# stdio2016/pfann

Measured on AMD Instinct MI355X. Metric: query segments/sec, 10 s @ SNR 0 queries vs 1M-segment db (exact flat IP top-100 + sequence match), higher is better.
Workload: dtype f32

## Files before the change

### pfann_amd/csrc/search_f16.hip

```cpp
#include "search_common.h"
#include <stdlib.h>

namespace pfann {

typedef _Float16 f16x8 __attribute__((ext_vector_type(8)));

__global__ void rows_to_half_kernel(const float *__restrict__ x, int64_t n, int d, _Float16 *__restrict__ xh,
                                    float *norm_max) {
    const int lane = threadIdx.x & 63;
    const int64_t row = (int64_t)blockIdx.x * (blockDim.x >> 6) + (threadIdx.x >> 6);
    if (row >= n) return;
    float ss = 0.f;
    for (int e = lane; e < d; e += 64) {
        const float v = x[row * d + e];
        xh[row * d + e] = (_Float16)v;
        ss = fmaf(v, v, ss);
    }
    ss = wave_sum(ss);
    if (lane == 0) atomicMax(reinterpret_cast<unsigned *>(norm_max), __float_as_uint(sqrtf(ss)));
}

int launch_rows_to_half(const float *x, int64_t n, int d, void *xh, float *norm_max_dev, hipStream_t s) {
    if (n <= 0) return 0;
    PF_LAUNCH(rows_to_half_kernel, dim3((unsigned)cdiv(n, 4)), dim3(256), 0, s, x, n, d,
// ... 46 lines not shown
    for (int i = tid; i < QT * BM; i += 256) {
        const int64_t m = (int64_t)mt0 * BM + i;
        thr_s[i] = dense ? 0.f : (m < p.nq ? -p.thr[m] : -INFINITY);
    }
    const char *qb = reinterpret_cast<const char *>(p.q), *dbb = reinterpret_cast<const char *>(p.db);
    const int64_t mq0 = (int64_t)mt0 * BM;
    const __amdgpu_buffer_rsrc_t srd_q = make_srd(qb + mq0 * row_bytes, (unsigned long long)(p.nq - mq0) * row_bytes);
    __amdgpu_buffer_rsrc_t srd_db[BR];
    unsigned doff[BR];
#pragma unroll
    for (int j = 0; j < BR; ++j) {
        const int64_t nj = n0 + 32 * j;
        const int64_t left = p.nrows - nj;
        srd_db[j] = make_srd(dbb + (nj < p.nrows ? nj : 0) * p.row_stride * row_bytes,
                             left > 0 ? (unsigned long long)((left - 1) * p.row_stride + 1) * row_bytes : 0ull);
        doff[j] = nj + rowq < p.nrows ? (unsigned)((unsigned long long)rowq * p.row_stride * row_bytes) : BUF_OOB;
    }
    f32x4 ra[AR], rb[BR];
    const int q_rows_left = (int)((p.nq - mq0) < (int64_t)QT * BM ? (p.nq - mq0) : (int64_t)QT * BM);
    const unsigned tile_bytes = (unsigned)BM * row_bytes;
    unsigned aoff[AR];
#pragma unroll
    for (int i = 0; i < AR; ++i) aoff[i] = (unsigned)(rowq + 32 * i) * row_bytes;
    unsigned lkb = (unsigned)col4 * 16u;
    int lrow = rowq;
    unsigned lbase = 0;
    auto load_tile = [&]() {
        const bool kok = lkb < row_bytes;
#pragma unroll
        for (int i = 0; i < AR; ++i)
            ra[i] = buf_load4(srd_q, (kok && lrow + 32 * i < q_rows_left) ? lbase + aoff[i] + lkb : BUF_OOB);
#pragma unroll
        for (int j = 0; j < BR; ++j) rb[j] = buf_load4(srd_db[j], (kok && doff[j] != BUF_OOB) ? doff[j] + lkb : BUF_OOB);
        lkb += 128u;
        const bool wrap = lkb >= row_bytes;
        lkb = wrap ? (unsigned)col4 * 16u : lkb;
        lrow += wrap ? BM : 0;
        lbase += wrap ? tile_bytes : 0u;
    };
    auto store_tile = [&](float *Ad, float *Bd) {
#pragma unroll
        for (int i = 0; i < AR; ++i)
            *reinterpret_cast<f32x4 *>(&Ad[(rowq + 32 * i) * LDK + col4 * 4]) = ra[i];
#pragma unroll
        for (int j = 0; j < BR; ++j)
            *reinterpret_cast<f32x4 *>(&Bd[(rowq + 32 * j) * LDK + col4 * 4]) = rb[j];
    };

    const int nk = (int)((row_bytes + 127u) / 128u);
    load_tile();
    store_tile(As, Bs);
    __syncthreads();
    const int l31 = lane & 31, lhalf = lane >> 5;
    int it = 0;
#pragma unroll 1
    for (int q = 0; q < n_q; ++q) {
        const int64_t m0 = mq0 + (int64_t)q * BM;
        const float *thr_c = thr_s + q * BM;
        f32x16 acc[TM][TN];
#pragma unroll
        for (int i = 0; i < TM; ++i)
#pragma unroll
            for (int g = 0; g < 4; ++g) {
                const f32x4 t4 = *reinterpret_cast<const f32x4 *>(thr_c + wm * WM + i * 32 + 8 * g + 4 * lhalf);
#pragma unroll
                for (int j = 0; j < TN; ++j)
#pragma unroll
                    for (int e = 0; e < 4; ++e) acc[i][j][4 * g + e] = t4[e];
            }
#pragma unroll 1
        for (int kt = 0; kt < nk; ++kt, ++it) {
            const float *Ac = As + (it & 1) * (BM * LDK), *Bc = Bs + (it & 1) * (BN * LDK);
            float *An = As + ((it + 1) & 1) * (BM * LDK), *Bn = Bs + ((it + 1) & 1) * (BN * LDK);
#pragma unroll
            for (int kk = 0; kk < 4; ++kk) {
                f16x8 a8[TM], b8[TN];
#pragma unroll
                for (int i = 0; i < TM; ++i)
                    a8[i] = __builtin_bit_cast(f16x8, *reinterpret_cast<const f32x4 *>(
                                                          &Ac[(wm * WM + i * 32 + l31) * LDK + kk * 8 + lhalf * 4]));
#pragma unroll
                for (int j = 0; j < TN; ++j)
                    b8[j] = __builtin_bit_cast(f16x8, *reinterpret_cast<const f32x4 *>(
                                                          &Bc[(wn * WN + j * 32 + l31) * LDK + kk * 8 + lhalf * 4]));
                if (kk == 0) {
                    load_tile();
                    __builtin_amdgcn_sched_barrier(0);
                }
                if (kk == 3) store_tile(An, Bn);
#pragma unroll
                for (int i = 0; i < TM; ++i)
#pragma unroll
                    for (int j = 0; j < TN; ++j)
                        acc[i][j] = __builtin_amdgcn_mfma_f32_32x32x16_f16(a8[i], b8[j], acc[i][j], 0, 0, 0);
            }
            __syncthreads();
        }
        if constexpr (EXCL) {
            if (excl_span_hit(p.excl_tile[m0 >> 7], n0 * p.row_stride, (n0 + BN - 1) * p.row_stride)) {
#pragma unroll
                for (int i = 0; i < TM; ++i)
#pragma unroll
                    for (int r = 0; r < 16; ++r) {
                        const int64_t m = m0 + wm * WM + i * 32 + (r & 3) + 8 * (r >> 2) + 4 * lhalf;
                        const uint2 ex = m < p.nq ? p.excl[m] : make_uint2(0u, 0u);
#pragma unroll
                        for (int j = 0; j < TN; ++j)
                            if (excl_hit(ex, (unsigned)((n0 + wn * WN + j * 32 + l31) * p.row_stride))) acc[i][j][r] = -INFINITY;
                    }
            }
        }
#pragma unroll
        for (int j = 0; j < TN; ++j) {
            const int64_t n = n0 + wn * WN + j * 32 + l31;
            const bool nok = n < p.nrows;
            const unsigned row = (unsigned)(n * p.row_stride);
#pragma unroll
            for (int i = 0; i < TM; ++i) {
                if (EXCL && dense) {
#pragma unroll
                    for (int r = 0; r < 16; ++r) {
                        const int64_t m = m0 + wm * WM + i * 32 + (r & 3) + 8 * (r >> 2) + 4 * lhalf;
                        if (nok && m < p.nq && acc[i][j][r] != -INFINITY)
                            p.keys[m * CAP + atomicAdd(&p.cnt[m], 1)] = pack_key(acc[i][j][r], row);
                    }
                } else if (dense) {
#pragma unroll
                    for (int r = 0; r < 16; ++r) {
                        const int64_t m = m0 + wm * WM + i * 32 + (r & 3) + 8 * (r >> 2) + 4 * lhalf;
                        if (nok && m < p.nq) p.keys[m * CAP + n] = pack_key(acc[i][j][r], row);
                    }
                } else {
                    float mx = fmaxf(acc[i][j][0], acc[i][j][1]);
#pragma unroll
                    for (int r = 2; r < 16; r += 2) mx = fmaxf(fmaxf(mx, acc[i][j][r]), acc[i][j][r + 1]);
                    if (__any(nok && mx >= 0.f)) {
#pragma unroll
                        for (int r = 0; r < 16; ++r) {
                            if (nok && acc[i][j][r] >= 0.f) {
                                const int ml = wm * WM + i * 32 + (r & 3) + 8 * (r >> 2) + 4 * lhalf;
                                const int64_t m = m0 + ml;
                                const int pos = atomicAdd(&p.cnt[m], 1);
                                if (pos < CAP) p.keys[m * CAP + pos] = pack_key(acc[i][j][r] - thr_c[ml], row);
                            }
                        }
                    }
                }
            }
        }
        __builtin_amdgcn_sched_barrier(0);
    }
}

#ifdef PFANN_SCAN_TRACE
__device__ unsigned long long *g_scan_trace = nullptr;
__device__ unsigned g_scan_trace_cap = 0;
#define SCAN_STAMP(i) do { const unsigned long long now_ = __builtin_readcyclecounter(); tr_sum[i] += now_ - tr_last; tr_last = now_; } while (0)
#else
#define SCAN_STAMP(i)
#endif

template <int KS, bool GMAX = false, int DBR = 128, int NBUF = 2, bool EXCL = false>
__global__ __launch_bounds__(256, DBR == 64 ? 3 : (NBUF == 3 ? 1 : 2)) void scan_f16_qres_kernel(ScanParams p) {
    constexpr int BM = 128, WM = 64, WN = DBR / 2, TM = 2, TN = WN / 32;
    constexpr bool BAL = !GMAX;
    constexpr int ROWB = KS * 32;
    constexpr int CPR = ROWB / 16;
    constexpr int NLD = DBR * CPR / 256;
    static_assert(!GMAX || DBR == 128, "the group-maximum pass assumes 64 groups per slice");
    constexpr int TILE_F = DBR * ROWB / 4, GS_F = GMAX ? BM * 64 : 0;
    __shared__ __attribute__((aligned(1024))) float Bs0[TILE_F > GS_F ? TILE_F : GS_F];
    __shared__ __attribute__((aligned(1024))) float Bs1[TILE_F];
    static_assert(NBUF == 2 || NBUF == 3, "two or three db-tile buffers");
    __shared__ __attribute__((aligned(1024))) float Bs2[NBUF == 3 ? TILE_F : 1];

    const int tid = threadIdx.x, lane = tid & 63, wave = tid >> 6;
    const int wm = wave >> 1, wn = wave & 1;
    const int l31 = lane & 31, lhalf = lane >> 5;
    const int S = p.nsub, subcap = CAP / (4 * S);
    const int L = xcd_remap(blockIdx.x, gridDim.x);
    const int seg = L / p.n_tiles_m, mt = L - seg * p.n_tiles_m;
    const int64_t m0 = (int64_t)mt * BM;
    const int64_t t_lo = seg, t_hi = (p.nrows + DBR - 1) / DBR;
    const __amdgpu_buffer_rsrc_t srd_k = make_srd(p.keys + m0 * CAP, (unsigned long long)BM * CAP * 8ull);
    const int own = 4 * seg + 2 * wn + lhalf;
    const unsigned own_off = (unsigned)(own * subcap) * 8u;
    int posr[TM];
#pragma unroll
    for (int i = 0; i < TM; ++i) posr[i] = 0;
    const char *qb = reinterpret_cast<const char *>(p.q), *dbb = reinterpret_cast<const char *>(p.db);
    uint2 ex_span = make_uint2(0xFFFFFFFFu, 0u);
    if constexpr (EXCL) ex_span = p.excl_tile[mt];

    const __amdgpu_buffer_rsrc_t srd_q = make_srd(qb + m0 * ROWB, (unsigned long long)(p.nq - m0) * ROWB);
    f16x8 afr[TM][KS];
#pragma unroll
    for (int i = 0; i < TM; ++i)
#pragma unroll
        for (int kk = 0; kk < KS; ++kk)
            afr[i][kk] = __builtin_bit_cast(f16x8, buf_load4(srd_q, (unsigned)(wm * WM + i * 32 + l31) * ROWB + kk * 32 + lhalf * 16));
    float th[TM];
#pragma unroll
    for (int i = 0; i < TM; ++i) {
        const int64_t m = m0 + wm * WM + i * 32 + l31;
        th[i] = GMAX ? 0.f : (m < p.nq ? p.thr[m] : INFINITY);
        if (EXCL && !GMAX) th[i] = fmaxf(th[i], -3.4028234663852886e38f);
    }
    f32x16 gmx[GMAX ? TM : 1][GMAX ? TN : 1];
#pragma unroll
    for (int i = 0; i < (GMAX ? TM : 1); ++i)
#pragma unroll
        for (int j = 0; j < (GMAX ? TN : 1); ++j)
#pragma unroll
            for (int r = 0; r < 16; ++r) gmx[i][j][r] = -INFINITY;
    f32x16 zero16;
#pragma unroll
    for (int r = 0; r < 16; ++r) zero16[r] = 0.f;
    constexpr int RP = 256 / ROWB;
    auto key = [](int r) { return BAL ? (((r >> 3) & 3) * (4 / RP)) | ((r & 3) / RP) : (r / RP) & (CPR - 1); };
    const int64_t rstride = DBR == 64 ? 1 : p.row_stride;
    const int64_t last_row = (p.nrows - 1) * rstride;
    unsigned goff[NLD];
    int lrow[NLD];
    const int wave_u = __builtin_amdgcn_readfirstlane(wave);
#pragma unroll
    for (int u = 0; u < NLD; ++u) {
        const int ci = (wave * NLD + u) * 64 + lane;
        const int r = ci / CPR, cs = ci % CPR;
        lrow[u] = r;
        goff[u] = (unsigned)((unsigned long long)r * (unsigned long long)rstride * ROWB) + (unsigned)((cs ^ key(r)) * 16);
    }
    auto load_tile = [&](int64_t t, float *Bd) {
        const int64_t r0 = t * DBR * rstride;
        const __amdgpu_buffer_rsrc_t srd_t = make_srd(dbb + r0 * ROWB, 0x7FFFFFF0ull);
        if ((t + 1) * DBR <= p.nrows) {
#pragma unroll
            for (int u = 0; u < NLD; ++u)
                __builtin_amdgcn_raw_ptr_buffer_load_lds(srd_t, (__attribute__((address_space(3))) void *)&Bd[(wave_u * NLD + u) * 256], 16,
                                                         (int)goff[u], 0, 0, 0);
        } else {
            const unsigned last_off = (unsigned)((last_row - r0) * ROWB);
#pragma unroll
            for (int u = 0; u < NLD; ++u) {
                const bool ok = t * DBR + lrow[u] < p.nrows;
                __builtin_amdgcn_raw_ptr_buffer_load_lds(srd_t, (__attribute__((address_space(3))) void *)&Bd[(wave_u * NLD + u) * 256], 16,
                                                         (int)(ok ? goff[u] : last_off + (goff[u] & (ROWB - 1))), 0, 0, 0);
            }
        }
    };
    if (t_lo < t_hi) load_tile(t_lo, Bs0);
    if (NBUF == 3 && t_lo + S < t_hi) {
        load_tile(t_lo + S, Bs1);
        asm volatile("s_waitcnt vmcnt(%0)\n\ts_waitcnt lgkmcnt(0)" :: "n"(NLD) : "memory");
        __builtin_amdgcn_s_barrier();
        asm volatile("" ::: "memory");
    } else {
        asm volatile("s_waitcnt vmcnt(0)" ::: "memory");
        __syncthreads();
    }
#ifdef PFANN_SCAN_TRACE
    unsigned long long tr_sum[5] = {0, 0, 0, 0, 0}, tr_last = __builtin_readcyclecounter(), tr_steps = 0;
#endif
    auto tile_step = [&](int64_t t, const float *Bc, float *Bn) {
        const bool req = t + (NBUF - 1) * S < t_hi;
        if (req) load_tile(t + (NBUF - 1) * S, Bn);
        __builtin_amdgcn_sched_barrier(0);
        SCAN_STAMP(0);
        f32x16 acc[TM][TN];
        constexpr int FA = 1;
        f16x8 b8[FA + 1][TN];
        auto frag = [&](int kk, int set) {
#pragma unroll
            for (int j = 0; j < TN; ++j) {
                const int r = BAL ? j * 64 + 8 * (l31 >> 2) + 4 * wn + (l31 & 3) : wn * WN + j * 32 + l31;
                b8[set][j] = __builtin_bit_cast(f16x8, *reinterpret_cast<const f32x4 *>(
                                                           &Bc[r * (ROWB / 4) + (((kk * 2 + lhalf) ^ key(r)) * 4)]));
            }
        };
#pragma unroll
        for (int kk = 0; kk < FA; ++kk) frag(kk, kk);
#pragma unroll
        for (int kk = 0; kk < KS; ++kk) {
            if (kk + FA < KS) frag(kk + FA, (kk + FA) % (FA + 1));
#pragma unroll
            for (int i = 0; i < TM; ++i)
#pragma unroll
                for (int j = 0; j < TN; ++j)
                    acc[i][j] = __builtin_amdgcn_mfma_f32_32x32x16_f16(b8[kk % (FA + 1)][j], afr[i][kk], kk == 0 ? zero16 : acc[i][j], 0, 0, 0);
            __builtin_amdgcn_sched_barrier(0);
        }
        SCAN_STAMP(1);
        if (NBUF == 3) {
            if (req) asm volatile("s_waitcnt vmcnt(%0)" :: "n"(NLD) : "memory");
            else asm volatile("s_waitcnt vmcnt(0)" ::: "memory");
        }
        const int nvalid = (int)(p.nrows - t * DBR < DBR ? p.nrows - t * DBR : DBR);
        if (nvalid < DBR) {
#pragma unroll
            for (int j = 0; j < TN; ++j)
#pragma unroll
                for (int r = 0; r < 16; ++r)
                    if ((BAL ? j * 64 + 16 * (r >> 2) + 8 * lhalf + 4 * wn + (r & 3) : wn * WN + j * 32 + 8 * (r >> 2) + 4 * lhalf + (r & 3)) >= nvalid) {
#pragma unroll
                        for (int i = 0; i < TM; ++i) acc[i][j][r] = -INFINITY;
                    }
        }
        if constexpr (EXCL) {
            if (excl_span_hit(ex_span, t * DBR * rstride, ((t + 1) * DBR - 1) * rstride)) {
#pragma unroll
                for (int i = 0; i < TM; ++i) {
                    const int64_t m = m0 + wm * WM + i * 32 + l31;
                    const uint2 ex = m < p.nq ? p.excl[m] : make_uint2(0u, 0u);
                    unsigned rs = (unsigned)rstride;
                    const unsigned len = ex.y - ex.x;
                    unsigned b0 = (unsigned)(t * DBR) * rs + (unsigned)(BAL ? 8 * lhalf + 4 * wn : wn * WN + 4 * lhalf) * rs - ex.x;
                    if constexpr (GMAX) {
                        asm volatile("" : "+s"(rs));
                        asm volatile("" : "+v"(b0));
                    }
#pragma unroll
                    for (int j = 0; j < TN; ++j)
#pragma unroll
                        for (int r = 0; r < 16; ++r) {
                            const int tr = BAL ? j * 64 + 16 * (r >> 2) + (r & 3) : j * 32 + 8 * (r >> 2) + (r & 3);
                            if (b0 + (unsigned)tr * rs < len) acc[i][j][r] = -INFINITY;
                        }
                }
            }
        }
#pragma unroll
        for (int j = 0; j < TN; ++j)
#pragma unroll
            for (int i = 0; i < TM; ++i) {
                float mg[4];
#pragma unroll
                for (int g = 0; g < 4; ++g)
                    mg[g] = fmaxf(fmaxf(acc[i][j][4 * g], acc[i][j][4 * g + 1]), fmaxf(acc[i][j][4 * g + 2], acc[i][j][4 * g + 3]));
                const float mx = fmaxf(fmaxf(mg[0], mg[1]), fmaxf(mg[2], mg[3]));
                if (GMAX) {
#pragma unroll
                    for (int r = 0; r < 16; ++r) gmx[i][j][r] = fmaxf(gmx[i][j][r], acc[i][j][r]);
                } else if (__any(mx >= th[i])) {
                    const int ml = wm * WM + i * 32 + l31;
                    const unsigned row0 = (unsigned)((t * DBR + j * 64 + 8 * lhalf + 4 * wn) * rstride);
                    int pos = posr[i];
#pragma unroll
                    for (int g = 0; g < 4; ++g) {
                        if (__any(mg[g] >= th[i])) {
#pragma unroll
                            for (int e = 0; e < 4; ++e) {
                                const float v = acc[i][j][4 * g + e];
                                const bool sv = v >= th[i];
                                const unsigned long long key = pack_key(v, row0 + (unsigned)((16 * g + e) * rstride));
                                typedef unsigned u32x2 __attribute__((ext_vector_type(2)));
                                __builtin_amdgcn_raw_buffer_store_b64(__builtin_bit_cast(u32x2, key), srd_k,
                                                                      (sv && pos < subcap) ? (unsigned)(ml * CAP + pos) * 8u + own_off : BUF_OOB, 0, 0);
                                pos += sv ? 1 : 0;
                            }
                        }
                    }
                    posr[i] = pos;
                }
            }
        SCAN_STAMP(2);
#ifdef PFANN_SCAN_TRACE
        ++tr_steps;
        if (NBUF == 2) {
            asm volatile("s_waitcnt vmcnt(0)" ::: "memory");
            SCAN_STAMP(3);
            __syncthreads();
            SCAN_STAMP(4);
        } else
#endif
        if (NBUF == 2) {
            asm volatile("s_waitcnt vmcnt(0)" ::: "memory");
            __syncthreads();
        } else {
            asm volatile("s_waitcnt lgkmcnt(0)" ::: "memory");
            __builtin_amdgcn_s_barrier();
            asm volatile("" ::: "memory");
        }
    };
    if constexpr (NBUF == 3) {
        int64_t t = t_lo;
#pragma unroll 1
        while (t < t_hi) {
            tile_step(t, Bs0, Bs2);
            t += S;
            if (t >= t_hi) break;
            __builtin_amdgcn_sched_barrier(0);
            tile_step(t, Bs1, Bs0);
            t += S;
            if (t >= t_hi) break;
            __builtin_amdgcn_sched_barrier(0);
            tile_step(t, Bs2, Bs1);
            t += S;
        }
    } else {
        int64_t t = t_lo;
#pragma unroll 1
        while (t < t_hi) {
            tile_step(t, Bs0, Bs1);
            t += S;
            if (t >= t_hi) break;
            __builtin_amdgcn_sched_barrier(0);
            tile_step(t, Bs1, Bs0);
            t += S;
        }
    }
    if constexpr (GMAX) {
        float *Gs = Bs0;
        static_assert(sizeof(Bs0) >= BM * 64 * sizeof(float), "group-maxima tile must fit its own LDS object");
#pragma unroll
        for (int i = 0; i < TM; ++i) {
            const int ml = wm * WM + i * 32 + l31;
#pragma unroll
            for (int j = 0; j < TN; ++j)
#pragma unroll
                for (int r = 0; r < 16; ++r) {
                    const float v = fmaxf(gmx[i][j][r], __shfl_xor(gmx[i][j][r], 32, 64));
                    const int slot = (wn * TN + j) * 16 + r;
                    if (lhalf == 0) Gs[ml * 64 + (slot ^ (ml & 31))] = v;
                }
        }
        __syncthreads();
        const int64_t G = (int64_t)S * 64;
        for (int it = 0; it < 8; ++it) {
            const int idx4 = it * 256 + tid, row = idx4 >> 4, c4 = idx4 & 15;
            f32x4 v;
#pragma unroll
            for (int e = 0; e < 4; ++e) v[e] = Gs[row * 64 + ((4 * c4 + e) ^ (row & 31))];
            if (m0 + row < p.nq) *reinterpret_cast<f32x4 *>(&p.gmax[(m0 + row) * G + seg * 64 + 4 * c4]) = v;
        }
        return;
    }
#pragma unroll
    for (int i = 0; i < TM; ++i) {
        const int64_t m = m0 + wm * WM + i * 32 + l31;
        if (m < p.nq) p.cnt[m * (4 * S) + own] = posr[i];
    }
#ifdef PFANN_SCAN_TRACE
    if (!GMAX && lane == 0 && g_scan_trace != nullptr && blockIdx.x < g_scan_trace_cap) {
        unsigned long long *o = g_scan_trace + ((size_t)blockIdx.x * 4 + wave) * 8;
        for (int i = 0; i < 5; ++i) o[i] = tr_sum[i];
        o[5] = tr_steps; o[6] = __builtin_amdgcn_s_getreg((31 << 11) | 4); o[7] = __builtin_amdgcn_s_getreg((31 << 11) | 20);
    }
#endif
}

#ifdef PFANN_SCAN_TRACE
extern "C" int pfann_debug_set_scan_trace(void *buf, unsigned cap_blocks) {
    if (hipMemcpyToSymbol(HIP_SYMBOL(g_scan_trace), &buf, sizeof(buf)) != hipSuccess) return -1;
    if (hipMemcpyToSymbol(HIP_SYMBOL(g_scan_trace_cap), &cap_blocks, sizeof(cap_blocks)) != hipSuccess) return -1;
    return 0;
}
#endif

__global__ void fill_int2_kernel(int *p, int v, int64_t n) {
    const int64_t i = (int64_t)blockIdx.x * blockDim.x + threadIdx.x;
    if (i < n) p[i] = v;
}

template <int NT>
__device__ __forceinline__ void sublist_offsets(const int *__restrict__ cnt_row, int nsub, int subcap, int *s_off, int *s_wt) {
    const int tid = threadIdx.x, lane = tid & 63, wave = tid >> 6;
    int incl = 0;
    bool ov = false;
    if (tid < NSUB_MAX) {
        int c = tid < nsub ? cnt_row[tid] : 0;
        ov = c > subcap;
        c = ov ? subcap : c;
        incl = c;
#pragma unroll
        for (int o = 1; o < 64; o <<= 1) {
            const int v = __shfl_up(incl, o, 64);
            if (lane >= o) incl += v;
        }
        if (lane == 63) s_wt[wave] = incl;
        const bool any_ov = __any(ov);
        if (lane == 0) s_wt[4 + wave] = any_ov ? 1 : 0;
    }
    __syncthreads();
    if (tid < NSUB_MAX) {
        int base = 0;
#pragma unroll
        for (int w = 0; w < 4; ++w) base += w < wave ? s_wt[w] : 0;
        s_off[tid + 1] = base + incl;
        if (tid == 0) {
            s_off[0] = 0;
            s_off[NSUB_MAX + 1] = s_wt[4] | s_wt[5] | s_wt[6] | s_wt[7];
        }
    }
    __syncthreads();
}


__device__ __forceinline__ float dense_canon_eps(const float *__restrict__ qv, int d, float xnorm_max) {
    float ss = 0.f;
    for (int e = 0; e < d; ++e) ss = fmaf(qv[e], qv[e], ss);
    return 2.f * (2.f * (d + 1) + 0.25f * d + 2.f) * 5.9604645e-8f * 1.001f * sqrtf(ss) * xnorm_max + 1e-36f * d;
}
__device__ __forceinline__ void select_rescore_small_row(const int64_t m, const unsigned long long *__restrict__ keys,
                                                const int *__restrict__ cnt, int k, int mode,
                                                float *__restrict__ thr, float *__restrict__ thr_adj,
                                                const float *__restrict__ eps, float *__restrict__ D,
                                                int64_t *__restrict__ I, int64_t label_base,
                                                int *overflow, int *__restrict__ row_ovf,
                                                const float *__restrict__ q32,
                                                const float *__restrict__ db32, int d, int nsub,
                                                int rescore, float dense_xn = -1.f) {
    constexpr int NT = 256, KPT = SMALL_N / NT;
    __shared__ __attribute__((aligned(16))) unsigned long long skeys[SMALL_N];
    __shared__ int s_n2, s_bin, s_kk;
    __shared__ int s_off[NSUB_MAX + 2], s_wt[8];
    __shared__ int hist[256];
    const int tid = threadIdx.x, lane = tid & 63, wave = tid >> 6;
    const int subcap = CAP / nsub;
    sublist_offsets<NT>(cnt + m * nsub, nsub, subcap, s_off, s_wt);
    const int n = s_off[nsub];
    if (n > SMALL_N) {
        if (tid == 0) atomicAdd(overflow + 1, 1);
        return;
    }
    const bool over = s_off[NSUB_MAX + 1] != 0;
    if (over && mode == 1 && tid == 0) row_ovf[m] = 1;
    if (nsub == 1) {
        for (int i = tid; i < n; i += NT) skeys[i] = keys[m * CAP + i];
    } else {
        const int l = tid & 7;
        for (int g = tid >> 3; g < nsub; g += NT / 8) {
            const int o = s_off[g], c = s_off[g + 1] - o;
            for (int i = l; i < c; i += 8) skeys[o + i] = keys[m * CAP + g * subcap + i];
        }
    }
    __syncthreads();
    const float e2 = rescore ? 2.0f * (dense_xn >= 0.f ? dense_canon_eps(q32 + m * d, d, dense_xn) : eps[m]) : 0.f;
    if (n <= k) {
        if (tid == 0) s_n2 = n;
        __syncthreads();
    } else {
        unsigned prefix = 0;
        int kk = k;
        for (int pass = 0; pass < 4; ++pass) {
            const int shift = 24 - 8 * pass;
            hist[tid] = 0;
            __syncthreads();
            for (int i = tid; i < n; i += NT) {
                const unsigned hi = (unsigned)(skeys[i] >> 32);
                if (pass == 0 || (hi >> (shift + 8)) == (prefix >> (shift + 8))) atomicAdd(&hist[(hi >> shift) & 255], 1);
            }
            __syncthreads();
            if (wave == 0) {
                const int c0 = hist[4 * lane], c1 = hist[4 * lane + 1], c2 = hist[4 * lane + 2], c3 = hist[4 * lane + 3];
                const int sum4 = c0 + c1 + c2 + c3;
                int incl = sum4;
#pragma unroll
                for (int o = 1; o < 64; o <<= 1) {
                    const int v = __shfl_up(incl, o, 64);
                    if (lane >= o) incl += v;
                }
                const int excl = incl - sum4;
                if (excl < kk && kk <= incl) {
                    int rem = kk - excl, bin = 4 * lane;
                    if (rem > c0) { rem -= c0; ++bin; if (rem > c1) { rem -= c1; ++bin; if (rem > c2) { rem -= c2; ++bin; } } }
                    s_bin = bin;
// ... 278 lines not shown
            for (int i = tid; i < n; i += 1024) {
                const unsigned hi = (unsigned)(skeys[i] >> 32);
                if (pass == 0 || (hi >> (shift + 8)) == (prefix >> (shift + 8))) atomicAdd(&hist[(hi >> shift) & 255], 1);
            }
            __syncthreads();
            if (wave == 0) {
                const int c0 = hist[4 * lane], c1 = hist[4 * lane + 1], c2 = hist[4 * lane + 2], c3 = hist[4 * lane + 3];
                const int sum4 = c0 + c1 + c2 + c3;
                int incl = sum4;
#pragma unroll
                for (int o = 1; o < 64; o <<= 1) {
                    const int v = __shfl_up(incl, o, 64);
                    if (lane >= o) incl += v;
                }
                const int excl = incl - sum4;
                if (excl < kk && kk <= incl) {
                    int rem = kk - excl, bin = 4 * lane;
                    if (rem > c0) { rem -= c0; ++bin; if (rem > c1) { rem -= c1; ++bin; if (rem > c2) { rem -= c2; ++bin; } } }
                    s_bin = bin;
                    s_kk = rem;
                }
            }
            __syncthreads();
            prefix |= (unsigned)s_bin << shift;
            kk = s_kk;
        }
        const float cut = ord2f(~prefix) - e2;
        const unsigned cut_hi = ~f2ord(cut);
        unsigned long long mine[KPT];
#pragma unroll
        for (int j = 0; j < KPT; ++j) mine[j] = tid + 1024 * j < n ? skeys[tid + 1024 * j] : ~0ull;
        if (tid == 0) s_n2 = 0;
        __syncthreads();
#pragma unroll
        for (int j = 0; j < KPT; ++j)
            if (tid + 1024 * j < n && (unsigned)(mine[j] >> 32) <= cut_hi) skeys[atomicAdd(&s_n2, 1)] = mine[j];
    }
    __syncthreads();
    const int n2 = s_n2;
    const float *qv = q32 + m * d;
    if (rescore)
    for (int c0 = 0; c0 < n2; c0 += 256) {
        const int c = c0 + (tid >> 2), sub = tid & 3;
        float part = 0.f;
        unsigned row = 0;
        if (c < n2) {
            row = (unsigned)(skeys[c] & 0xFFFFFFFFull);
            part = canon_part(db32 + (int64_t)row * d, qv, d, sub);
        }
        part = canon_sum(part);
        if (c < n2 && sub == 0) skeys[c] = pack_key(part, row);
    }
    __syncthreads();
    if (n2 <= 1024) {
        unsigned long long mine = ~0ull;
        int rank = 0;
        if (tid < n2) {
            mine = skeys[tid];
            for (int j = 0; j < n2; ++j) rank += skeys[j] < mine ? 1 : 0;
        }
        __syncthreads();
        if (tid < n2) skeys[rank] = mine;
        __syncthreads();
    } else {
        int P2 = 1;
        while (P2 < n2) P2 <<= 1;
        for (int i = n2 + tid; i < P2; i += 1024) skeys[i] = ~0ull;
        __syncthreads();
        bitonic_sort_u64(skeys, P2, tid, 1024);
    }
    if (mode == 0) {
        if (tid == 0) {
            const float t = n2 >= k ? ord2f(~(unsigned)(skeys[k - 1] >> 32)) : -INFINITY;
            thr[m] = t;
            thr_adj[m] = fmaxf(rescore ? t - eps[m] : t, -1000.f * eps[m]);
        }
    } else {
        for (int i = tid; i < k; i += 1024) {
            if (i < n2) {
                const unsigned long long key = skeys[i];
                D[m * k + i] = ord2f(~(unsigned)(key >> 32));
                I[m * k + i] = (int64_t)(unsigned)(key & 0xFFFFFFFFu) + label_base;
            } else {
                D[m * k + i] = -3.4028234663852886e38f;
                I[m * k + i] = -1;
            }
        }
    }
}

__global__ __launch_bounds__(1024) void select_rescore_kernel(const unsigned long long *__restrict__ keys,
                                                              const int *__restrict__ cnt, int k, int mode,
                                                              float *__restrict__ thr, float *__restrict__ thr_adj,
                                                              const float *__restrict__ eps, float *__restrict__ D,
                                                              int64_t *__restrict__ I, int64_t label_base,
                                                              int *overflow, int *__restrict__ row_ovf,
                                                              const float *__restrict__ q32,
                                                              const float *__restrict__ db32, int d, int nsub,
                                                              int rescore) {
    select_rescore_body(keys, cnt, k, mode, thr, thr_adj, eps, D, I, label_base, overflow, row_ovf, q32, db32, d, nsub, rescore);
}

__global__ __launch_bounds__(1024) void select_rescore_list_kernel(const unsigned long long *__restrict__ keys,
                                                                   const int *__restrict__ cnt, int k, int mode,
                                                                   float *__restrict__ thr, float *__restrict__ thr_adj,
                                                                   const float *__restrict__ eps, float *__restrict__ D,
                                                                   int64_t *__restrict__ I, int64_t label_base,
                                                                   int *overflow, int *__restrict__ row_ovf,
                                                                   const float *__restrict__ q32,
                                                                   const float *__restrict__ db32, int d, int nsub,
                                                                   int rescore, const int *__restrict__ left) {
    if (overflow[1] == 0) return;
    const int n_left = overflow[2];
    for (int it = blockIdx.x; it < n_left; it += gridDim.x) {
        select_rescore_body(keys, cnt, k, mode, thr, thr_adj, eps, D, I, label_base, overflow, row_ovf, q32, db32, d, nsub, rescore, left[it]);
        __syncthreads();
    }
}

__global__ __launch_bounds__(256) void select_dense_small_kernel(const unsigned long long *__restrict__ keys, const int *__restrict__ cnt,
                                                                 int k, float *D, int64_t *I, int64_t label_base, int *overflow,
                                                                 int *row_ovf, const float *__restrict__ q32,
                                                                 const float *__restrict__ db32, int d, float xnorm_max) {
    select_rescore_small_row(blockIdx.x, keys, cnt, k, 1, nullptr, nullptr, nullptr, D, I, label_base, overflow, row_ovf, q32, db32, d, 1, 1,
                             xnorm_max);
}
__global__ __launch_bounds__(1024) void select_dense_kernel(const unsigned long long *__restrict__ keys, const int *__restrict__ cnt, int k,
                                                            float *D, int64_t *I, int64_t label_base, int *overflow, int *row_ovf,
                                                            const float *__restrict__ q32, const float *__restrict__ db32, int d,
                                                            float xnorm_max) {
    select_rescore_body(keys, cnt, k, 1, nullptr, nullptr, nullptr, D, I, label_base, overflow, row_ovf, q32, db32, d, 1, 1, -1,
                        xnorm_max);
}

template <int FB_ELT, bool EXCL = false>
__global__ __launch_bounds__(1024) void select_tail_kernel(const unsigned long long *__restrict__ keys, const int *__restrict__ cnt, int k,
                                                           float *__restrict__ thr, float *__restrict__ thr_adj,
                                                           const float *__restrict__ eps, float *D, int64_t *I, int64_t label_base,
                                                           int *overflow, int *row_ovf, const float *__restrict__ q32,
                                                           const float *__restrict__ db32, int d, int nsub, int rescore,
                                                           const void *__restrict__ fb_rows, int64_t n,
                                                           const uint2 *__restrict__ excl) {
    select_rescore_body(keys, cnt, k, 1, thr, thr_adj, eps, D, I, label_base, overflow, row_ovf, q32, db32, d, nsub, rescore);
    __syncthreads();
    topk_fallback_body<FB_ELT, 1024, EXCL>(blockIdx.x, row_ovf, q32, fb_rows, n, d, k, D, I, label_base, excl);
}

int launch_stage_f16(const SearchStage &st, const StageArgs &a) {
    SearchWorkspace &ws = a.ws;
    hipStream_t s = a.s;
    const dim3 grid(st.grid), block(st.block);
    const unsigned long long *keys = reinterpret_cast<const unsigned long long *>(ws.cl);
    const float *db32 = a.db32(st);
    switch (st.kernel) {
#define X(id, ...) case K_##id: PF_LAUNCH((__VA_ARGS__), grid, block, st.lds, s, scan_params(st, a)); break;
    PF_SCAN_F16_KERNELS(X) PF_SCAN_F16_EXCL_KERNELS(X)
#undef X
    case K_Q_PREP:
        PF_LAUNCH(q_prep_kernel, grid, block, 0, s, a.q, a.nq, a.d, a.xnorm_max, reinterpret_cast<_Float16 *>(ws.qh), ws.eps, ws.row_ovf);
        break;
    case K_FILL_INT2: PF_LAUNCH(fill_int2_kernel, grid, block, 0, s, ws.cnt, st.fill, a.nq); break;
    case K_SELECT_RESCORE_SMALL:
        PF_LAUNCH(select_rescore_small_kernel, grid, block, 0, s, keys, ws.cnt, a.k, st.mode, ws.thr, ws.thr_adj, ws.eps, a.D, a.I,
                  a.label_base, ws.overflow, ws.row_ovf, a.q, db32, a.d, st.nsub, st.rescore);
        break;
    case K_SELECT_RESCORE:
        if (ensure_dyn_lds((const void *)select_rescore_kernel, CAP * 8)) return -1;
        PF_LAUNCH(select_rescore_kernel, grid, block, st.lds, s, keys, ws.cnt, a.k, st.mode, ws.thr, ws.thr_adj, ws.eps, a.D, a.I,
                  a.label_base, ws.overflow, ws.row_ovf, a.q, db32, a.d, st.nsub, st.rescore);
        break;
    case K_SELECT_RESCORE_WAVE:
        PF_LAUNCH(select_rescore_wave_kernel, grid, block, 0, s, keys, ws.cnt, a.k, ws.eps, a.D, a.I, a.label_base, ws.overflow, a.q, db32,
                  a.d, st.nsub, st.rescore, a.nq, ws.left);
        break;
    case K_SELECT_RESCORE_SMALL_LIST:
        PF_LAUNCH(select_rescore_small_list_kernel, grid, block, 0, s, keys, ws.cnt, a.k, st.mode, ws.thr, ws.thr_adj, ws.eps, a.D, a.I,
                  a.label_base, ws.overflow, ws.row_ovf, a.q, db32, a.d, st.nsub, st.rescore, ws.left);
        break;
    case K_SELECT_RESCORE_LIST:
        if (ensure_dyn_lds((const void *)select_rescore_list_kernel, CAP * 8)) return -1;
        PF_LAUNCH(select_rescore_list_kernel, grid, block, st.lds, s, keys, ws.cnt, a.k, st.mode, ws.thr, ws.thr_adj, ws.eps, a.D, a.I,
                  a.label_base, ws.overflow, ws.row_ovf, a.q, db32, a.d, st.nsub, st.rescore, ws.left);
        break;
    case K_SELECT_DENSE_SMALL:
        PF_LAUNCH(select_dense_small_kernel, grid, block, 0, s, keys, ws.cnt, a.k, a.D, a.I, a.label_base, ws.overflow, ws.row_ovf, a.q, a.db,
                  a.d, a.xnorm_max > 0.f ? a.xnorm_max : 0.f);
        break;
    case K_SELECT_DENSE:
        if (ensure_dyn_lds((const void *)select_dense_kernel, CAP * 8)) return -1;
        PF_LAUNCH(select_dense_kernel, grid, block, st.lds, s, keys, ws.cnt, a.k, a.D, a.I, a.label_base, ws.overflow, ws.row_ovf, a.q, a.db,
                  a.d, a.xnorm_max > 0.f ? a.xnorm_max : 0.f);
        break;
    case K_SELECT_TAIL_4:
        if (ensure_dyn_lds((const void *)select_tail_kernel<4>, CAP * 8)) return -1;
        PF_LAUNCH(select_tail_kernel<4>, grid, block, st.lds, s, keys, ws.cnt, a.k, ws.thr, ws.thr_adj, ws.eps, a.D, a.I, a.label_base,
                  ws.overflow, ws.row_ovf, a.q, db32, a.d, st.nsub, st.rescore, (const void *)a.db, a.n, (const uint2 *)nullptr);
        break;
    case K_SELECT_TAIL_4_EXCL:
        if (ensure_dyn_lds((const void *)select_tail_kernel<4, true>, CAP * 8)) return -1;
        PF_LAUNCH((select_tail_kernel<4, true>), grid, block, st.lds, s, keys, ws.cnt, a.k, ws.thr, ws.thr_adj, ws.eps, a.D, a.I, a.label_base,
                  ws.overflow, ws.row_ovf, a.q, db32, a.d, st.nsub, st.rescore, (const void *)a.db, a.n, (const uint2 *)ws.excl);
        break;
    case K_SELECT_TAIL_2_EXCL:
        if (ensure_dyn_lds((const void *)select_tail_kernel<2, true>, CAP * 8)) return -1;
        PF_LAUNCH((select_tail_kernel<2, true>), grid, block, st.lds, s, keys, ws.cnt, a.k, ws.thr, ws.thr_adj, ws.eps, a.D, a.I, a.label_base,
                  ws.overflow, ws.row_ovf, a.q, db32, a.d, st.nsub, st.rescore, a.dbh, a.n, (const uint2 *)ws.excl);
        break;
    case K_SELECT_TAIL_2:
        if (ensure_dyn_lds((const void *)select_tail_kernel<2>, CAP * 8)) return -1;
        PF_LAUNCH(select_tail_kernel<2>, grid, block, st.lds, s, keys, ws.cnt, a.k, ws.thr, ws.thr_adj, ws.eps, a.D, a.I, a.label_base,
                  ws.overflow, ws.row_ovf, a.q, db32, a.d, st.nsub, st.rescore, a.dbh, a.n, (const uint2 *)nullptr);
        break;
    default: set_error("search: stage with unknown kernel %d", st.kernel); return -1;
    }
    PF_HIP(hipGetLastError());
    return 0;
}

__global__ void noop_search_f16_kernel() {}
int prewarm_search_f16() {
    hipLaunchKernelGGL(noop_search_f16_kernel, dim3(1), dim3(1), 0, 0);
    return hipGetLastError() == hipSuccess ? 0 : -1;
}

}
```

Baseline: 228,000.

## Restructure scan tile loop to process one column block at a time

```diff
diff --git a/pfann_amd/csrc/search_f16.hip b/pfann_amd/csrc/search_f16.hip
--- a/pfann_amd/csrc/search_f16.hip
+++ b/pfann_amd/csrc/search_f16.hip
@@ -222,6 +222,9 @@
     }
 }
 
+#ifndef PFANN_SCAN_EARLY_BARRIER
+#define PFANN_SCAN_EARLY_BARRIER 0
+#endif
 #ifdef PFANN_SCAN_TRACE
 __device__ unsigned long long *g_scan_trace = nullptr;
 __device__ unsigned g_scan_trace_cap = 0;
@@ -237,6 +240,7 @@
     constexpr int ROWB = KS * 32;
     constexpr int CPR = ROWB / 16;
     constexpr int NLD = DBR * CPR / 256;
+    constexpr bool EARLY_BAR = PFANN_SCAN_EARLY_BARRIER && NBUF == 2 && !GMAX && TN == 1;
     static_assert(!GMAX || DBR == 128, "the group-maximum pass assumes 64 groups per slice");
     constexpr int TILE_F = DBR * ROWB / 4, GS_F = GMAX ? BM * 64 : 0;
     __shared__ __attribute__((aligned(1024))) float Bs0[TILE_F > GS_F ? TILE_F : GS_F];
@@ -287,17 +291,15 @@
 #pragma unroll
     for (int r = 0; r < 16; ++r) zero16[r] = 0.f;
     constexpr int RP = 256 / ROWB;
-    auto key = [](int r) { return BAL ? (((r >> 3) & 3) * (4 / RP)) | ((r & 3) / RP) : (r / RP) & (CPR - 1); };
+    constexpr auto key = [](int r) constexpr { return BAL ? (((r >> 3) & 3) * (4 / RP)) | ((r & 3) / RP) : (r / RP) & (CPR - 1); };
     const int64_t rstride = DBR == 64 ? 1 : p.row_stride;
     const int64_t last_row = (p.nrows - 1) * rstride;
     unsigned goff[NLD];
-    int lrow[NLD];
     const int wave_u = __builtin_amdgcn_readfirstlane(wave);
 #pragma unroll
     for (int u = 0; u < NLD; ++u) {
         const int ci = (wave * NLD + u) * 64 + lane;
         const int r = ci / CPR, cs = ci % CPR;
-        lrow[u] = r;
         goff[u] = (unsigned)((unsigned long long)r * (unsigned long long)rstride * ROWB) + (unsigned)((cs ^ key(r)) * 16);
     }
     auto load_tile = [&](int64_t t, float *Bd) {
@@ -310,11 +312,15 @@
                                                          (int)goff[u], 0, 0, 0);
         } else {
             const unsigned last_off = (unsigned)((last_row - r0) * ROWB);
+            int lane_o = lane;
+            asm volatile("" : "+v"(lane_o));
 #pragma unroll
             for (int u = 0; u < NLD; ++u) {
-                const bool ok = t * DBR + lrow[u] < p.nrows;
+                const bool ok = t * DBR + ((wave_u * NLD + u) * 64 + lane_o) / CPR < p.nrows;
+                unsigned go = goff[u];
+                asm volatile("" : "+v"(go));
                 __builtin_amdgcn_raw_ptr_buffer_load_lds(srd_t, (__attribute__((address_space(3))) void *)&Bd[(wave_u * NLD + u) * 256], 16,
-                                                         (int)(ok ? goff[u] : last_off + (goff[u] & (ROWB - 1))), 0, 0, 0);
+                                                         (int)(ok ? goff[u] : last_off + (go & (ROWB - 1))), 0, 0, 0);
             }
         }
     };
@@ -336,81 +342,90 @@
         if (req) load_tile(t + (NBUF - 1) * S, Bn);
         __builtin_amdgcn_sched_barrier(0);
         SCAN_STAMP(0);
-        f32x16 acc[TM][TN];
         constexpr int FA = 1;
-        f16x8 b8[FA + 1][TN];
-        auto frag = [&](int kk, int set) {
-#pragma unroll
-            for (int j = 0; j < TN; ++j) {
-                const int r = BAL ? j * 64 + 8 * (l31 >> 2) + 4 * wn + (l31 & 3) : wn * WN + j * 32 + l31;
-                b8[set][j] = __builtin_bit_cast(f16x8, *reinterpret_cast<const f32x4 *>(
-                                                           &Bc[r * (ROWB / 4) + (((kk * 2 + lhalf) ^ key(r)) * 4)]));
-            }
+        f16x8 b8[FA + 1];
+        constexpr int BROWS = BAL ? 64 : 32;
+        const int fr = BAL ? 8 * (l31 >> 2) + 4 * wn + (l31 & 3) : wn * WN + l31;
+        static_assert(TN == 1 || key(5) == key(BROWS + 5), "a block's fragment rows keep the swizzle key of block 0");
+        auto frag = [&](int s) {
+            const int j = s / KS, kk = s % KS;
+            b8[s % (FA + 1)] = __builtin_bit_cast(f16x8, *reinterpret_cast<const f32x4 *>(
+                                                             &Bc[fr * (ROWB / 4) + (((kk * 2 + lhalf) ^ key(fr)) * 4) + j * BROWS * (ROWB / 4)]));
         };
-#pragma unroll
-        for (int kk = 0; kk < FA; ++kk) frag(kk, kk);
-#pragma unroll
-        for (int kk = 0; kk < KS; ++kk) {
-            if (kk + FA < KS) frag(kk + FA, (kk + FA) % (FA + 1));
-#pragma unroll
-            for (int i = 0; i < TM; ++i)
-#pragma unroll
-                for (int j = 0; j < TN; ++j)
-                    acc[i][j] = __builtin_amdgcn_mfma_f32_32x32x16_f16(b8[kk % (FA + 1)][j], afr[i][kk], kk == 0 ? zero16 : acc[i][j], 0, 0, 0);
-            __builtin_amdgcn_sched_barrier(0);
-        }
-        SCAN_STAMP(1);
-        if (NBUF == 3) {
-            if (req) asm volatile("s_waitcnt vmcnt(%0)" :: "n"(NLD) : "memory");
-            else asm volatile("s_waitcnt vmcnt(0)" ::: "memory");
-        }
         const int nvalid = (int)(p.nrows - t * DBR < DBR ? p.nrows - t * DBR : DBR);
-        if (nvalid < DBR) {
-#pragma unroll
-            for (int j = 0; j < TN; ++j)
+        f32x16 acc[TN > 1 ? 2 : 1][TM];
+        auto fold = [&](int i, int j) {
+#pragma unroll
+            for (int r = 0; r < 16; ++r) gmx[GMAX ? i : 0][GMAX ? j : 0][r] = fmaxf(gmx[GMAX ? i : 0][GMAX ? j : 0][r], acc[j & 1][i][r]);
+            asm volatile("" : "+v"(gmx[GMAX ? i : 0][GMAX ? j : 0]));
+        };
+#pragma unroll
+        for (int s = 0; s < FA; ++s) frag(s);
+#pragma unroll
+        for (int j = 0; j < TN; ++j) {
+#pragma unroll
+            for (int kk = 0; kk < KS; ++kk) {
+                if (j * KS + kk + FA < TN * KS) frag(j * KS + kk + FA);
+#pragma unroll
+                for (int i = 0; i < TM; ++i)
+                    acc[j & 1][i] = __builtin_amdgcn_mfma_f32_32x32x16_f16(b8[(j * KS + kk) % (FA + 1)], afr[i][kk], kk == 0 ? zero16 : acc[j & 1][i], 0, 0, 0);
+                if (GMAX && j > 0 && kk >= 1 && kk <= TM) fold(kk - 1, j - 1);
+                __builtin_amdgcn_sched_barrier(0);
+            }
+            SCAN_STAMP(1);
+            if (NBUF == 3 && j == (GMAX ? TN - 1 : 0)) {
+                if (req) asm volatile("s_waitcnt vmcnt(%0)" :: "n"(NLD) : "memory");
+                else asm volatile("s_waitcnt vmcnt(0)" ::: "memory");
+            }
+            if (EARLY_BAR) {
+                asm volatile("s_waitcnt vmcnt(0)" ::: "memory");
+                SCAN_STAMP(3);
+                __syncthreads();
+                SCAN_STAMP(4);
+            }
+            if (nvalid < DBR) {
+                int lim = nvalid - (BAL ? 8 * lhalf + 4 * wn : wn * WN + 4 * lhalf);
+                asm volatile("" : "+v"(lim));
 #pragma unroll
                 for (int r = 0; r < 16; ++r)
-                    if ((BAL ? j * 64 + 16 * (r >> 2) + 8 * lhalf + 4 * wn + (r & 3) : wn * WN + j * 32 + 8 * (r >> 2) + 4 * lhalf + (r & 3)) >= nvalid) {
-#pragma unroll
-                        for (int i = 0; i < TM; ++i) acc[i][j][r] = -INFINITY;
+                    if ((BAL ? j * 64 + 16 * (r >> 2) + (r & 3) : j * 32 + 8 * (r >> 2) + (r & 3)) >= lim) {
+#pragma unroll
+                        for (int i = 0; i < TM; ++i) acc[j & 1][i][r] = -INFINITY;
                     }
-        }
-        if constexpr (EXCL) {
-            if (excl_span_hit(ex_span, t * DBR * rstride, ((t + 1) * DBR - 1) * rstride)) {
-#pragma unroll
-                for (int i = 0; i < TM; ++i) {
-                    const int64_t m = m0 + wm * WM + i * 32 + l31;
-                    const uint2 ex = m < p.nq ? p.excl[m] : make_uint2(0u, 0u);
-                    unsigned rs = (unsigned)rstride;
-                    const unsigned len = ex.y - ex.x;
-                    unsigned b0 = (unsigned)(t * DBR) * rs + (unsigned)(BAL ? 8 * lhalf + 4 * wn : wn * WN + 4 * lhalf) * rs - ex.x;
-                    if constexpr (GMAX) {
-                        asm volatile("" : "+s"(rs));
-                        asm volatile("" : "+v"(b0));
-                    }
-#pragma unroll
-                    for (int j = 0; j < TN; ++j)
+            }
+            if constexpr (EXCL) {
+                if (excl_span_hit(ex_span, t * DBR * rstride, ((t + 1) * DBR - 1) * rstride)) {
+#pragma unroll
+                    for (int i = 0; i < TM; ++i) {
+                        const int64_t m = m0 + wm * WM + i * 32 + l31;
+                        const uint2 ex = m < p.nq ? p.excl[m] : make_uint2(0u, 0u);
+                        unsigned rs = (unsigned)rstride;
+                        const unsigned len = ex.y - ex.x;
+                        unsigned b0 = (unsigned)(t * DBR) * rs + (unsigned)(BAL ? 8 * lhalf + 4 * wn : wn * WN + 4 * lhalf) * rs - ex.x;
+                        if constexpr (GMAX) {
+                            asm volatile("" : "+s"(rs));
+                            asm volatile("" : "+v"(b0));
+                        }
 #pragma unroll
                         for (int r = 0; r < 16; ++r) {
                             const int tr = BAL ? j * 64 + 16 * (r >> 2) + (r & 3) : j * 32 + 8 * (r >> 2) + (r & 3);
-                            if (b0 + (unsigned)tr * rs < len) acc[i][j][r] = -INFINITY;
+                            if (b0 + (unsigned)tr * rs < len) acc[j & 1][i][r] = -INFINITY;
                         }
+                    }
                 }
             }
-        }
-#pragma unroll
-        for (int j = 0; j < TN; ++j)
 #pragma unroll
             for (int i = 0; i < TM; ++i) {
+                if (GMAX) {
+                    if (j == TN - 1) fold(i, j);
+                    continue;
+                }
                 float mg[4];
 #pragma unroll
                 for (int g = 0; g < 4; ++g)
-                    mg[g] = fmaxf(fmaxf(acc[i][j][4 * g], acc[i][j][4 * g + 1]), fmaxf(acc[i][j][4 * g + 2], acc[i][j][4 * g + 3]));
+                    mg[g] = fmaxf(fmaxf(acc[j & 1][i][4 * g], acc[j & 1][i][4 * g + 1]), fmaxf(acc[j & 1][i][4 * g + 2], acc[j & 1][i][4 * g + 3]));
                 const float mx = fmaxf(fmaxf(mg[0], mg[1]), fmaxf(mg[2], mg[3]));
-                if (GMAX) {
-#pragma unroll
-                    for (int r = 0; r < 16; ++r) gmx[i][j][r] = fmaxf(gmx[i][j][r], acc[i][j][r]);
-                } else if (__any(mx >= th[i])) {
+                if (__any(mx >= th[i])) {
                     const int ml = wm * WM + i * 32 + l31;
                     const unsigned row0 = (unsigned)((t * DBR + j * 64 + 8 * lhalf + 4 * wn) * rstride);
                     int pos = posr[i];
@@ -419,7 +434,7 @@
                         if (__any(mg[g] >= th[i])) {
 #pragma unroll
                             for (int e = 0; e < 4; ++e) {
-                                const float v = acc[i][j][4 * g + e];
+                                const float v = acc[j & 1][i][4 * g + e];
                                 const bool sv = v >= th[i];
                                 const unsigned long long key = pack_key(v, row0 + (unsigned)((16 * g + e) * rstride));
                                 typedef unsigned u32x2 __attribute__((ext_vector_type(2)));
@@ -432,19 +447,17 @@
                     posr[i] = pos;
                 }
             }
+        }
         SCAN_STAMP(2);
 #ifdef PFANN_SCAN_TRACE
         ++tr_steps;
-        if (NBUF == 2) {
+#endif
+        if (EARLY_BAR) {
+        } else if (NBUF == 2) {
             asm volatile("s_waitcnt vmcnt(0)" ::: "memory");
             SCAN_STAMP(3);
             __syncthreads();
             SCAN_STAMP(4);
-        } else
-#endif
-        if (NBUF == 2) {
-            asm volatile("s_waitcnt vmcnt(0)" ::: "memory");
-            __syncthreads();
         } else {
             asm volatile("s_waitcnt lgkmcnt(0)" ::: "memory");
             __builtin_amdgcn_s_barrier();
```

After: 228,300, median of 2. About the same (+0.1%).

## Stream per-column MFMA accumulators into group maxima to cut GMAX register pressure

Applied to the files above, without the earlier changes.

```diff
diff --git a/pfann_amd/csrc/search_f16.hip b/pfann_amd/csrc/search_f16.hip
--- a/pfann_amd/csrc/search_f16.hip
+++ b/pfann_amd/csrc/search_f16.hip
@@ -291,37 +291,43 @@
     const int64_t rstride = DBR == 64 ? 1 : p.row_stride;
     const int64_t last_row = (p.nrows - 1) * rstride;
     unsigned goff[NLD];
-    int lrow[NLD];
+    constexpr int RPI = 64 / CPR;
+    const int lrow0 = wave * NLD * RPI + lane / CPR;
     const int wave_u = __builtin_amdgcn_readfirstlane(wave);
 #pragma unroll
     for (int u = 0; u < NLD; ++u) {
         const int ci = (wave * NLD + u) * 64 + lane;
         const int r = ci / CPR, cs = ci % CPR;
-        lrow[u] = r;
         goff[u] = (unsigned)((unsigned long long)r * (unsigned long long)rstride * ROWB) + (unsigned)((cs ^ key(r)) * 16);
     }
+    constexpr int LD_WHOLE = NLD, LD_RAGGED = NLD, VM_TILE = NLD;
+    static_assert(LD_WHOLE == VM_TILE && LD_RAGGED == VM_TILE, "vmcnt of the three-buffer waits = loads per tile request, in both load_tile branches");
+    static_assert(VM_TILE >= 1 && VM_TILE <= 63, "vmcnt is a 6-bit field");
     auto load_tile = [&](int64_t t, float *Bd) {
         const int64_t r0 = t * DBR * rstride;
         const __amdgpu_buffer_rsrc_t srd_t = make_srd(dbb + r0 * ROWB, 0x7FFFFFF0ull);
         if ((t + 1) * DBR <= p.nrows) {
 #pragma unroll
-            for (int u = 0; u < NLD; ++u)
+            for (int u = 0; u < LD_WHOLE; ++u)
                 __builtin_amdgcn_raw_ptr_buffer_load_lds(srd_t, (__attribute__((address_space(3))) void *)&Bd[(wave_u * NLD + u) * 256], 16,
                                                          (int)goff[u], 0, 0, 0);
         } else {
             const unsigned last_off = (unsigned)((last_row - r0) * ROWB);
-#pragma unroll
-            for (int u = 0; u < NLD; ++u) {
-                const bool ok = t * DBR + lrow[u] < p.nrows;
+            const int nleft = (int)(p.nrows - t * DBR);
+#pragma unroll
+            for (int u = 0; u < LD_RAGGED; ++u) {
+                const bool ok = lrow0 + u * RPI < nleft;
+                unsigned g = goff[u];
+                asm volatile("" : "+v"(g));
                 __builtin_amdgcn_raw_ptr_buffer_load_lds(srd_t, (__attribute__((address_space(3))) void *)&Bd[(wave_u * NLD + u) * 256], 16,
-                                                         (int)(ok ? goff[u] : last_off + (goff[u] & (ROWB - 1))), 0, 0, 0);
+                                                         (int)(ok ? g : last_off + (g & (ROWB - 1))), 0, 0, 0);
             }
         }
     };
     if (t_lo < t_hi) load_tile(t_lo, Bs0);
     if (NBUF == 3 && t_lo + S < t_hi) {
         load_tile(t_lo + S, Bs1);
-        asm volatile("s_waitcnt vmcnt(%0)\n\ts_waitcnt lgkmcnt(0)" :: "n"(NLD) : "memory");
+        asm volatile("s_waitcnt vmcnt(%0)\n\ts_waitcnt lgkmcnt(0)" :: "n"(VM_TILE) : "memory");
         __builtin_amdgcn_s_barrier();
         asm volatile("" ::: "memory");
     } else {
@@ -336,7 +342,58 @@
         if (req) load_tile(t + (NBUF - 1) * S, Bn);
         __builtin_amdgcn_sched_barrier(0);
         SCAN_STAMP(0);
-        f32x16 acc[TM][TN];
+        const int nvalid = (int)(p.nrows - t * DBR < DBR ? p.nrows - t * DBR : DBR);
+        constexpr int TNA = GMAX ? 1 : TN;
+        f32x16 acc[TM][TNA];
+        auto fold = [&](int i, int j) {
+            if (nvalid < DBR) {
+                int nv = nvalid - (wn * WN + j * 32 + 4 * lhalf);
+                asm volatile("" : "+v"(nv));
+#pragma unroll
+                for (int r = 0; r < 16; ++r)
+                    if (8 * (r >> 2) + (r & 3) >= nv) acc[i][0][r] = -INFINITY;
+            }
+            if constexpr (EXCL) {
+                if (excl_span_hit(ex_span, t * DBR * rstride, ((t + 1) * DBR - 1) * rstride)) {
+                    int ml = wm * WM + i * 32 + l31;
+                    asm volatile("" : "+v"(ml));
+                    const int64_t m = m0 + ml;
+                    const uint2 ex = m < p.nq ? p.excl[m] : make_uint2(0u, 0u);
+                    unsigned rs = (unsigned)rstride;
+                    const unsigned len = ex.y - ex.x;
+                    unsigned b0 = (unsigned)(t * DBR) * rs + (unsigned)(wn * WN + j * 32 + 4 * lhalf) * rs - ex.x;
+                    asm volatile("" : "+s"(rs));
+                    asm volatile("" : "+v"(b0));
+#pragma unroll
+                    for (int r = 0; r < 16; ++r)
+                        if (b0 + (unsigned)(8 * (r >> 2) + (r & 3)) * rs < len) acc[i][0][r] = -INFINITY;
+                }
+            }
+#pragma unroll
+            for (int r = 0; r < 16; ++r) gmx[GMAX ? i : 0][GMAX ? j : 0][r] = fmaxf(gmx[GMAX ? i : 0][GMAX ? j : 0][r], acc[i][0][r]);
+        };
+        if constexpr (GMAX) {
+            constexpr int FG = 3, NS = TN * KS;
+            f16x8 b8[FG + 1];
+            auto frag = [&](int s) {
+                const int r = wn * WN + (s / KS) * 32 + l31;
+                b8[s % (FG + 1)] = __builtin_bit_cast(f16x8, *reinterpret_cast<const f32x4 *>(
+                                                                 &Bc[r * (ROWB / 4) + ((((s % KS) * 2 + lhalf) ^ key(r)) * 4)]));
+            };
+#pragma unroll
+            for (int s = 0; s < FG && s < NS; ++s) frag(s);
+#pragma unroll
+            for (int s = 0; s < NS; ++s) {
+                const int j = s / KS, kk = s % KS;
+                if (s + FG < NS) frag(s + FG);
+#pragma unroll
+                for (int i = 0; i < TM; ++i) {
+                    if (kk == 0 && j > 0) fold(i, j - 1);
+                    acc[i][0] = __builtin_amdgcn_mfma_f32_32x32x16_f16(b8[s % (FG + 1)], afr[i][kk], kk == 0 ? zero16 : acc[i][0], 0, 0, 0);
+                }
+                __builtin_amdgcn_sched_barrier(0);
+            }
+        } else {
         constexpr int FA = 1;
         f16x8 b8[FA + 1][TN];
         auto frag = [&](int kk, int set) {
@@ -355,22 +412,29 @@
 #pragma unroll
             for (int i = 0; i < TM; ++i)
 #pragma unroll
-                for (int j = 0; j < TN; ++j)
+                for (int j = 0; j < TNA; ++j)
                     acc[i][j] = __builtin_amdgcn_mfma_f32_32x32x16_f16(b8[kk % (FA + 1)][j], afr[i][kk], kk == 0 ? zero16 : acc[i][j], 0, 0, 0);
             __builtin_amdgcn_sched_barrier(0);
         }
+        }
         SCAN_STAMP(1);
         if (NBUF == 3) {
-            if (req) asm volatile("s_waitcnt vmcnt(%0)" :: "n"(NLD) : "memory");
+            if (req) asm volatile("s_waitcnt vmcnt(%0)" :: "n"(VM_TILE) : "memory");
             else asm volatile("s_waitcnt vmcnt(0)" ::: "memory");
         }
-        const int nvalid = (int)(p.nrows - t * DBR < DBR ? p.nrows - t * DBR : DBR);
+        if constexpr (GMAX) {
+#pragma unroll
+            for (int i = 0; i < TM; ++i) fold(i, TN - 1);
+        } else {
+        static_assert(BAL, "the survivor epilogue assumes the balanced mapping");
         if (nvalid < DBR) {
+            int nv = nvalid - (8 * lhalf + 4 * wn);
+            asm volatile("" : "+v"(nv));
 #pragma unroll
             for (int j = 0; j < TN; ++j)
 #pragma unroll
                 for (int r = 0; r < 16; ++r)
-                    if ((BAL ? j * 64 + 16 * (r >> 2) + 8 * lhalf + 4 * wn + (r & 3) : wn * WN + j * 32 + 8 * (r >> 2) + 4 * lhalf + (r & 3)) >= nvalid) {
+                    if (j * 64 + 16 * (r >> 2) + (r & 3) >= nv) {
 #pragma unroll
                         for (int i = 0; i < TM; ++i) acc[i][j][r] = -INFINITY;
                     }
@@ -383,16 +447,12 @@
                     const uint2 ex = m < p.nq ? p.excl[m] : make_uint2(0u, 0u);
                     unsigned rs = (unsigned)rstride;
                     const unsigned len = ex.y - ex.x;
-                    unsigned b0 = (unsigned)(t * DBR) * rs + (unsigned)(BAL ? 8 * lhalf + 4 * wn : wn * WN + 4 * lhalf) * rs - ex.x;
-                    if constexpr (GMAX) {
-                        asm volatile("" : "+s"(rs));
-                        asm volatile("" : "+v"(b0));
-                    }
+                    unsigned b0 = (unsigned)(t * DBR) * rs + (unsigned)(8 * lhalf + 4 * wn) * rs - ex.x;
 #pragma unroll
                     for (int j = 0; j < TN; ++j)
 #pragma unroll
                         for (int r = 0; r < 16; ++r) {
-                            const int tr = BAL ? j * 64 + 16 * (r >> 2) + (r & 3) : j * 32 + 8 * (r >> 2) + (r & 3);
+                            const int tr = j * 64 + 16 * (r >> 2) + (r & 3);
                             if (b0 + (unsigned)tr * rs < len) acc[i][j][r] = -INFINITY;
                         }
                 }
@@ -407,10 +467,7 @@
                 for (int g = 0; g < 4; ++g)
                     mg[g] = fmaxf(fmaxf(acc[i][j][4 * g], acc[i][j][4 * g + 1]), fmaxf(acc[i][j][4 * g + 2], acc[i][j][4 * g + 3]));
                 const float mx = fmaxf(fmaxf(mg[0], mg[1]), fmaxf(mg[2], mg[3]));
-                if (GMAX) {
-#pragma unroll
-                    for (int r = 0; r < 16; ++r) gmx[i][j][r] = fmaxf(gmx[i][j][r], acc[i][j][r]);
-                } else if (__any(mx >= th[i])) {
+                if (__any(mx >= th[i])) {
                     const int ml = wm * WM + i * 32 + l31;
                     const unsigned row0 = (unsigned)((t * DBR + j * 64 + 8 * lhalf + 4 * wn) * rstride);
                     int pos = posr[i];
@@ -432,6 +489,7 @@
                     posr[i] = pos;
                 }
             }
+        }
         SCAN_STAMP(2);
 #ifdef PFANN_SCAN_TRACE
         ++tr_steps;
@@ -481,6 +539,9 @@
     if constexpr (GMAX) {
         float *Gs = Bs0;
         static_assert(sizeof(Bs0) >= BM * 64 * sizeof(float), "group-maxima tile must fit its own LDS object");
+        int tid_e = threadIdx.x;
+        asm volatile("" : "+v"(tid_e));
+        const int tid = tid_e, lane = tid & 63, wave = tid >> 6, wm = wave >> 1, wn = wave & 1, l31 = lane & 31, lhalf = lane >> 5;
 #pragma unroll
         for (int i = 0; i < TM; ++i) {
             const int ml = wm * WM + i * 32 + l31;
@@ -1065,6 +1126,16 @@
     const dim3 grid(st.grid), block(st.block);
     const unsigned long long *keys = reinterpret_cast<const unsigned long long *>(ws.cl);
     const float *db32 = a.db32(st);
+    switch (st.kernel) {
+    case K_QRES_8_DBR64_NBUF3: case K_QRES_8_DBR64: case K_QRES_8: case K_QRES_4:
+    case K_QRES_8_DBR64_NBUF3_EXCL: case K_QRES_8_DBR64_EXCL: case K_QRES_8_EXCL: case K_QRES_4_EXCL:
+        if (st.nsub < 1 || 4 * st.nsub > NSUB_MAX) {
+            set_error("search: query-stationary full pass with %d slices (4 lists each, at most %d)", st.nsub, NSUB_MAX);
+            return -1;
+        }
+        break;
+    default: break;
+    }
     switch (st.kernel) {
 #define X(id, ...) case K_##id: PF_LAUNCH((__VA_ARGS__), grid, block, st.lds, s, scan_params(st, a)); break;
     PF_SCAN_F16_KERNELS(X) PF_SCAN_F16_EXCL_KERNELS(X)
```

Measured after the change: 229,400 before, 230,100 after, median of 3. About the same (+0.3%).
